# gnss-sdr/gnss-sdr

Hardware: NVIDIA B200
Metric: Msamples/s through N-channel E/P/L correlator (higher is better)
Workload: dtype f32

## Files before the change

### gnss_sdr_b200/csrc/trk_shared_kernel.cu

```cuda
#include "trk_device.cuh"

namespace b200
{
constexpr int kShK = 8;
constexpr int kShTile = 512;
#ifndef SH_STAGES
#define SH_STAGES 4
#endif
#ifndef SH_MINB
#define SH_MINB 3
#endif
constexpr int kShStages = SH_STAGES;
#ifndef SH_STRESS
#define SH_STRESS 0
#endif
#if SH_STRESS
__device__ __forceinline__ void stress_delay(unsigned int salt)
{
    unsigned int h = salt * 2654435761u;
    h ^= h >> 15;
    h *= 2246822519u;
    h ^= h >> 13;
    if ((h & 3u) == 0u) __nanosleep(100u + ((h >> 4) & 1023u));
}
#endif
constexpr int kShTblCap = 1152;
constexpr int kShWin = 256;
constexpr int kShThreads = (kShK + 1) * 32;
constexpr int kShReseed = 64;

namespace
{
struct __align__(128) ShSmem
{
    float2 tiles[kShStages][kShTile];
    float tbl[kShK][kShTblCap];
    unsigned long long full[kShStages];
    unsigned long long empty[kShStages];
    unsigned long long item_start[kShK];
    int item_n[kShK];
    int item_band[kShK];
    unsigned long long hull_start;
    int n_tiles;
    int share;
};

__device__ __forceinline__ unsigned int smem_u32(const void* p) { return static_cast<unsigned int>(__cvta_generic_to_shared(p)); }

__device__ __forceinline__ void mbar_init(unsigned long long* bar, unsigned int count)
{
    asm volatile("mbarrier.init.shared::cta.b64 [%0], %1;" ::"r"(smem_u32(bar)), "r"(count) : "memory");
}
__device__ __forceinline__ void mbar_arrive(unsigned long long* bar)
{
    asm volatile("mbarrier.arrive.shared::cta.b64 _, [%0];" ::"r"(smem_u32(bar)) : "memory");
}
__device__ __forceinline__ void mbar_arrive_expect_tx(unsigned long long* bar, unsigned int bytes)
{
    asm volatile("mbarrier.arrive.expect_tx.shared::cta.b64 _, [%0], %1;" ::"r"(smem_u32(bar)), "r"(bytes) : "memory");
}
__device__ __forceinline__ void mbar_wait(unsigned long long* bar, unsigned int parity)
{
    asm volatile(
        "{\n\t"
        ".reg .pred P1;\n\t"
        "LAB_WAIT:\n\t"
        "mbarrier.try_wait.parity.shared::cta.b64 P1, [%0], %1, %2;\n\t"
        "@P1 bra DONE;\n\t"
        "bra LAB_WAIT;\n\t"
        "DONE:\n\t"
        "}" ::"r"(smem_u32(bar)),
        "r"(parity), "r"(0x989680u)
        : "memory");
}
__device__ __forceinline__ void bulk_g2s(void* smem_dst, const void* gmem_src, unsigned int bytes, unsigned long long* bar)
{
    asm volatile("cp.async.bulk.shared::cluster.global.mbarrier::complete_tx::bytes [%0], [%1], %2, [%3];" ::"r"(smem_u32(smem_dst)),
                 "l"(gmem_src), "r"(bytes), "r"(smem_u32(bar))
                 : "memory");
}

template <int TAPS>
__device__ void warp_correlate_general(const b200_trk_item& it, const ChanDesc& ch, const BandDesc& bd, float2 (&acc)[TAPS])
{
    const int lane = threadIdx.x & 31;
    const unsigned long long s0 = it.sample_index - bd.first_index;
    const unsigned long long T0 = turns_from_rad(-static_cast<double>(it.rem_carrier_phase_rad));
    const unsigned long long DT = turns_from_rad(-static_cast<double>(it.phase_step_rad));
    const int body = (it.n / 8) * 8;
    for (int n = lane; n < it.n; n += 32)
        {
            const float2 x = ldg_stream8(bd.base + ((s0 + static_cast<unsigned long long>(n)) & bd.mask));
            const float2 z = phasor_from_turns(T0 + DT * static_cast<unsigned long long>(n));
            const float wr = fmaf(x.x, z.x, -x.y * z.y);
            const float wi = fmaf(x.x, z.y, x.y * z.x);
            const float nf = static_cast<float>(n);
#pragma unroll
            for (int t = 0; t < TAPS; t++)
                {
                    const int idx = (n < body) ? chip_index_avx(it.code_phase_step_chips, nf, __fsub_rn(ch.shifts[t], it.rem_code_phase_chips))
                                               : chip_index_generic(it.code_phase_step_chips, nf, ch.shifts[t], it.rem_code_phase_chips);
                    const float c = ch.code[mod_pos(idx, ch.code_len)];
                    acc[t].x = fmaf(wr, c, acc[t].x);
                    acc[t].y = fmaf(wi, c, acc[t].y);
                }
        }
}

struct SmemTileLoader
{
    const float4* p;
    __device__ __forceinline__ float4 operator()(int k) const { return p[32 * k]; }
};
struct GlobalTileLoader
{
    const float2* base;
    unsigned long long mask, off, limit;
    __device__ __forceinline__ float4 operator()(int k) const
    {
        const unsigned long long o = off + 64ULL * static_cast<unsigned long long>(k);
        if (mask == ~0ULL && o + 2ULL > limit) return make_float4(0.f, 0.f, 0.f, 0.f);
        return ldg_stream16(base + (o & mask));
    }
};

template <int TAPS, bool MASKED, class Loader>
__device__ __forceinline__ void warp_tile(const Loader& load, float vlo, float vhi, float step, const float2 (&aux2)[TAPS],
    unsigned int tbl_off, float2 Dr2, float2 Di2, float& fa, float& fb, float2& zr, float2& zi, float2 (&are)[TAPS], float2 (&aim)[TAPS])
{
    const float2 magic2 = make_float2(12582912.0f, 12582912.0f);
#pragma unroll
    for (int k = 0; k < kShTile / 64; k++)
        {
            const float4 v = load(k);
            float ua = fa, ub = fb;
            float2 xa = make_float2(v.x, v.y), xb = make_float2(v.z, v.w);
            if (MASKED)
                {
                    if (fa < vlo || fa > vhi) xa = make_float2(0.f, 0.f);
                    if (fb < vlo || fb > vhi) xb = make_float2(0.f, 0.f);
                    ua = fminf(fmaxf(fa, vlo), vhi);
                    ub = fminf(fmaxf(fb, vlo), vhi);
                }
            float2 wr2, wi2;
            wr2.x = fmaf(xa.x, zr.x, -xa.y * zi.x);
            wi2.x = fmaf(xa.x, zi.x, xa.y * zr.x);
            wr2.y = fmaf(xb.x, zr.y, -xb.y * zi.y);
            wi2.y = fmaf(xb.x, zi.y, xb.y * zr.y);
            const float2 m2 = make_float2(__fmul_rn(step, ua), __fmul_rn(step, ub));
#pragma unroll
            for (int t = 0; t < TAPS; t++)
                {
                    const float2 tt = __fadd2_rd(__fadd2_rn(m2, aux2[t]), magic2);
                    const float ca = lds_f32((__float_as_uint(tt.x) << 2) + tbl_off);
                    const float cb = lds_f32((__float_as_uint(tt.y) << 2) + tbl_off);
                    const float2 c2 = make_float2(ca, cb);
                    are[t] = __ffma2_rn(wr2, c2, are[t]);
                    aim[t] = __ffma2_rn(wi2, c2, aim[t]);
                }
            const float2 t1 = __fmul2_rn(zi, Di2);
            const float2 nzr = __ffma2_rn(zr, Dr2, make_float2(-t1.x, -t1.y));
            zi = __ffma2_rn(zr, Di2, __fmul2_rn(zi, Dr2));
            zr = nzr;
            fa += 64.0f;
            fb += 64.0f;
        }
}

template <int TAPS>
__global__ void __launch_bounds__(kShThreads, SH_MINB) trk_shared_kernel(const b200_trk_item* __restrict__ items, int n_items,
    const ChanDesc* __restrict__ chans, const BandDesc* __restrict__ bands, float2* __restrict__ out, int out_stride)
{
    extern __shared__ __align__(128) unsigned char sh_raw[];
    ShSmem& sm = *reinterpret_cast<ShSmem*>(sh_raw);
    const int warp = threadIdx.x >> 5, lane = threadIdx.x & 31;
    const int group = blockIdx.x;
    const int item_id = group * kShK + warp;
    const bool consumer = warp < kShK;
    const bool have_item = consumer && item_id < n_items;

    b200_trk_item it;
    ChanDesc const* ch = nullptr;
    BandDesc bd;
    if (have_item)
        {
            it = items[item_id];
            ch = &chans[it.channel];
            bd = bands[ch->band];
        }
    if (threadIdx.x == 0)
        {
            for (int s = 0; s < kShStages; s++)
                {
                    mbar_init(&sm.full[s], 1);
                    mbar_init(&sm.empty[s], kShK);
                }
            asm volatile("fence.mbarrier_init.release.cluster;" ::: "memory");
        }
    if (consumer && lane == 0)
        {
            sm.item_n[warp] = have_item ? it.n : 0;
            sm.item_band[warp] = have_item ? ch->band : -1;
            sm.item_start[warp] = have_item ? (it.sample_index - bd.first_index) : 0ULL;
        }
    __syncthreads();
    if (threadIdx.x == 0)
        {
            unsigned long long lo = ~0ULL, hi = 0ULL;
            int band = -1, share = 1, nmax = 0;
            for (int w = 0; w < kShK; w++)
                {
                    if (sm.item_n[w] <= 0) continue;
                    if (band < 0) band = sm.item_band[w];
                    if (sm.item_band[w] != band) share = 0;
                    lo = min(lo, sm.item_start[w]);
                    hi = max(hi, sm.item_start[w] + static_cast<unsigned long long>(sm.item_n[w]));
                    nmax = max(nmax, sm.item_n[w]);
                }
            if (band < 0) share = 0;
            lo &= ~1ULL;
            if (share && (hi - lo) > 3ULL * static_cast<unsigned long long>(nmax) + 2ULL * kShTile) share = 0;
            sm.hull_start = lo;
            sm.n_tiles = share ? static_cast<int>((hi - lo + kShTile - 1) / kShTile) : 0;
            sm.share = share;
        }
    __syncthreads();
    const int n_tiles = sm.n_tiles;
    const unsigned long long hull_start = sm.hull_start;

    if (!consumer)
        {
            if (lane == 0 && n_tiles > 0)
                {
                    BandDesc pb;
                    {
                        int w0 = 0;
                        while (sm.item_n[w0] <= 0) w0++;
                        pb = bands[sm.item_band[w0]];
                    }
                    const bool ring = (pb.mask != ~0ULL);
                    const unsigned long long cap = ring ? pb.mask + 1ULL : pb.limit;
                    for (int t = 0; t < n_tiles; t++)
                        {
                            const int s = t % kShStages;
                            const unsigned int par = static_cast<unsigned int>((t / kShStages) & 1);
                            mbar_wait(&sm.empty[s], par ^ 1u);
#if SH_STRESS
                            stress_delay(static_cast<unsigned int>(t) * 31u + blockIdx.x * 7u + 3u);
#endif
                            unsigned long long src = hull_start + static_cast<unsigned long long>(t) * kShTile;
                            unsigned int n1 = kShTile, n2 = 0;
                            if (ring)
                                {
                                    src &= pb.mask;
                                    if (src + kShTile > cap)
                                        {
                                            n1 = static_cast<unsigned int>(cap - src);
                                            n2 = kShTile - n1;
                                        }
                                }
                            else
                                {
                                    if (src >= cap)
                                        n1 = 0;
                                    else if (src + kShTile > cap)
                                        n1 = static_cast<unsigned int>(cap - src) & ~1u;
                                }
                            mbar_arrive_expect_tx(&sm.full[s], (n1 + n2) * 8u);
                            if (n1) bulk_g2s(&sm.tiles[s][0], pb.base + src, n1 * 8u, &sm.full[s]);
                            if (n2) bulk_g2s(&sm.tiles[s][n1], pb.base, n2 * 8u, &sm.full[s]);
                        }
                }
            return;
        }

    float2 acc[TAPS];
#pragma unroll
    for (int t = 0; t < TAPS; t++) acc[t] = make_float2(0.f, 0.f);

    bool table_path = false, whole_table = false;
    unsigned long long my_hull = 0;
    int body = 0, a_i = 0, t_first = 0, t_last = 0;
    float step = 0.f;
    unsigned int tbl_off = 0;
    float2 aux2[TAPS];
    float2 Dr2, Di2, Gr2, Gi2, zr2, zi2, zr, zi;
    unsigned long long T0 = 0, DT = 0;
    if (have_item && it.n > 0)
        {
            body = (it.n / 8) * 8;
            step = it.code_phase_step_chips;
            const float rem = it.rem_code_phase_chips;
            T0 = turns_from_rad(-static_cast<double>(it.rem_carrier_phase_rad));
            DT = turns_from_rad(-static_cast<double>(it.phase_step_rad));
            float smin = ch->shifts[0], smax = ch->shifts[0];
#pragma unroll
            for (int t = 0; t < TAPS; t++)
                {
                    const float sh = ch->shifts[t];
                    const float a2 = __fsub_rn(sh, rem);
                    aux2[t] = make_float2(a2, a2);
                    smin = fminf(smin, sh);
                    smax = fmaxf(smax, sh);
                }
            const float span_bound = ceilf(fabsf(step) * static_cast<float>(kShTile)) + ceilf(smax - smin) + 6.0f;
            table_path = !ch->high_dyn && span_bound <= static_cast<float>(kShWin) && fabsf(step) * static_cast<float>(it.n) < 3.0e6f &&
                         fabsf(smax) < 1.0e5f && fabsf(smin) < 1.0e5f && fabsf(rem) < 1.0e6f;
            if (table_path)
                {
                    {
                        int elo = 0x7fffffff, ehi = -0x7fffffff - 1;
                        const float nl = static_cast<float>(max(body - 1, 0));
#pragma unroll
                        for (int q = 0; q < TAPS; q++)
                            {
                                const int i0 = chip_index_avx(step, 0.f, aux2[q].x);
                                const int i1 = chip_index_avx(step, nl, aux2[q].x);
                                elo = min(elo, min(i0, i1));
                                ehi = max(ehi, max(i0, i1));
                            }
                        whole_table = (static_cast<long long>(ehi) - elo + 3) <= kShTblCap;
                        if (whole_table)
                            {
                                const int wb = elo - 1;
                                const int wspan = ehi - elo + 3;
                                const int L = ch->code_len;
                                int r = mod_pos(wb + lane, L);
                                const int stride = 32 % L;
                                for (int j = lane; j < wspan; j += 32)
                                    {
                                        sm.tbl[warp][j] = __ldg(ch->code + r);
                                        r += stride;
                                        if (r >= L) r -= L;
                                    }
                                asm("sub.u32 %0, %1, %2;" : "=r"(tbl_off) : "r"(smem_u32(&sm.tbl[warp][0])), "r"(4u * (static_cast<unsigned int>(wb) + 0x4B400000u)));
                                __syncwarp();
                            }
                    }
                    my_hull = sm.share ? hull_start : (sm.item_start[warp] & ~1ULL);
                    a_i = static_cast<int>(sm.item_start[warp] - my_hull);
                    t_first = a_i / kShTile;
                    t_last = (a_i + body + kShTile - 1) / kShTile;
                    const float2 D = phasor_from_turns(DT * 64ULL);
                    const float2 G = phasor_from_turns(DT * static_cast<unsigned long long>(64 * kShReseed));
                    Dr2 = make_float2(D.x, D.x);
                    Di2 = make_float2(D.y, D.y);
                    Gr2 = make_float2(G.x, G.x);
                    Gi2 = make_float2(G.y, G.y);
                    const long long n0 = static_cast<long long>(t_first) * kShTile + 2 * lane - a_i;
                    const float2 za = phasor_from_turns(T0 + DT * static_cast<unsigned long long>(n0));
                    const float2 zb = phasor_from_turns(T0 + DT * static_cast<unsigned long long>(n0 + 1));
                    zr2 = make_float2(za.x, zb.x);
                    zi2 = make_float2(za.y, zb.y);
                    zr = zr2;
                    zi = zi2;
                }
        }

    float2 are[TAPS], aim[TAPS];
#pragma unroll
    for (int t = 0; t < TAPS; t++) are[t] = aim[t] = make_float2(0.f, 0.f);
    int tiles_in_group = 0;
    int next_wb = 0;
    float fa = static_cast<float>(t_first * kShTile + 2 * lane - a_i), fb = fa + 1.0f;
    auto process_tile = [&](int t, const auto& load) {
        const int n_tile0 = t * kShTile - a_i;
        const bool interior = (n_tile0 >= 0) && (n_tile0 + kShTile <= body);
        const int n_lo = max(n_tile0, 0), n_hi = min(n_tile0 + kShTile, body) - 1;
        const float vlo = static_cast<float>(n_lo), vhi = static_cast<float>(n_hi);
        if (!whole_table)
            {
                auto stage_window = [&](int tt) {
                    const int m0 = tt * kShTile - a_i;
                    const float lo_f = static_cast<float>(max(m0, 0)), hi_f = static_cast<float>(min(m0 + kShTile, body) - 1);
                    int wlo = 0x7fffffff, whi = -0x7fffffff - 1;
#pragma unroll
                    for (int q = 0; q < TAPS; q++)
                        {
                            const int i0 = chip_index_avx(step, lo_f, aux2[q].x);
                            const int i1 = chip_index_avx(step, hi_f, aux2[q].x);
                            wlo = min(wlo, min(i0, i1));
                            whi = max(whi, max(i0, i1));
                        }
                    const int wb = wlo - 1;
                    const int wspan = min(whi - wlo + 3, kShWin);
                    const int L = ch->code_len;
                    int r = mod_pos(wb + lane, L);
                    const int stride = 32 % L;
                    float* dst = &sm.tbl[warp][(tt & 1) * kShWin];
                    for (int j = lane; j < wspan; j += 32)
                        {
                            asm volatile("cp.async.ca.shared.global [%0], [%1], 4;" ::"r"(smem_u32(dst + j)), "l"(ch->code + r) : "memory");
                            r += stride;
                            if (r >= L) r -= L;
                        }
                    return wb;
                };
                if (t == t_first) next_wb = stage_window(t);
                const int wb = next_wb;
                asm volatile("cp.async.wait_all;" ::: "memory");
                __syncwarp();
                if (t + 1 < t_last) next_wb = stage_window(t + 1);
                asm("sub.u32 %0, %1, %2;" : "=r"(tbl_off) : "r"(smem_u32(&sm.tbl[warp][(t & 1) * kShWin])), "r"(4u * (static_cast<unsigned int>(wb) + 0x4B400000u)));
            }
        if (interior)
            warp_tile<TAPS, false>(load, vlo, vhi, step, aux2, tbl_off, Dr2, Di2, fa, fb, zr, zi, are, aim);
        else
            warp_tile<TAPS, true>(load, vlo, vhi, step, aux2, tbl_off, Dr2, Di2, fa, fb, zr, zi, are, aim);
        if (++tiles_in_group == kShReseed / 8)
            {
                const float2 t2 = __fmul2_rn(zi2, Gi2);
                const float2 ngr = __ffma2_rn(zr2, Gr2, make_float2(-t2.x, -t2.y));
                zi2 = __ffma2_rn(zr2, Gi2, __fmul2_rn(zi2, Gr2));
                zr2 = ngr;
                zr = zr2;
                zi = zi2;
                tiles_in_group = 0;
            }
        __syncwarp();
    };

    for (int t = 0; t < n_tiles; t++)
        {
            const int s = t % kShStages;
            const unsigned int par = static_cast<unsigned int>((t / kShStages) & 1);
            mbar_wait(&sm.full[s], par);
#if SH_STRESS
            stress_delay(static_cast<unsigned int>(t) * 17u + static_cast<unsigned int>(warp) * 101u + blockIdx.x * 13u);
#endif
            if (table_path && t >= t_first && t < t_last)
                {
                    const SmemTileLoader ld{reinterpret_cast<const float4*>(&sm.tiles[s][0]) + lane};
                    process_tile(t, ld);
                }
#if SH_STRESS
            stress_delay(static_cast<unsigned int>(t) * 29u + static_cast<unsigned int>(warp) * 53u + blockIdx.x * 5u + 1u);
            __syncwarp();
#endif
            if (lane == 0) mbar_arrive(&sm.empty[s]);
        }
    if (!sm.share && table_path)
        {
            for (int t = t_first; t < t_last; t++)
                {
                    const GlobalTileLoader ld{bd.base, bd.mask, my_hull + static_cast<unsigned long long>(t) * kShTile + 2ULL * lane, bd.limit};
                    process_tile(t, ld);
                }
        }
    if (have_item && it.n > 0)
        {
            if (table_path)
                {
#pragma unroll
                    for (int t = 0; t < TAPS; t++)
                        {
                            acc[t].x = are[t].x + are[t].y;
                            acc[t].y = aim[t].x + aim[t].y;
                        }
                    const int n = body + lane;
                    if (n < it.n)
                        {
                            const unsigned long long s0 = it.sample_index - bd.first_index;
                            const float2 x = ldg_stream8(bd.base + ((s0 + static_cast<unsigned long long>(n)) & bd.mask));
                            const float2 z = phasor_from_turns(T0 + DT * static_cast<unsigned long long>(n));
                            const float wr = fmaf(x.x, z.x, -x.y * z.y);
                            const float wi = fmaf(x.x, z.y, x.y * z.x);
#pragma unroll
                            for (int t = 0; t < TAPS; t++)
                                {
                                    const int idx = chip_index_generic(step, static_cast<float>(n), ch->shifts[t], it.rem_code_phase_chips);
                                    const float c = __ldg(ch->code + mod_pos(idx, ch->code_len));
                                    acc[t].x = fmaf(wr, c, acc[t].x);
                                    acc[t].y = fmaf(wi, c, acc[t].y);
                                }
                        }
                }
            else
                {
                    warp_correlate_general<TAPS>(it, *ch, bd, acc);
                }
#pragma unroll
            for (int t = 0; t < TAPS; t++)
                {
#pragma unroll
                    for (int o = 16; o > 0; o >>= 1)
                        {
                            acc[t].x += __shfl_xor_sync(0xffffffffu, acc[t].x, o);
                            acc[t].y += __shfl_xor_sync(0xffffffffu, acc[t].y, o);
                        }
                }
            if (lane < TAPS)
                {
                    float2 r = acc[0];
#pragma unroll
                    for (int t = 1; t < TAPS; t++)
                        if (lane == t) r = acc[t];
                    out[static_cast<size_t>(item_id) * out_stride + lane] = r;
                }
        }
    else if (have_item && lane < ch->taps)
        {
            out[static_cast<size_t>(item_id) * out_stride + lane] = make_float2(0.f, 0.f);
        }
}
}

int launch_trk_shared(const b200_trk_item* items, int n_items, const ChanDesc* chans, const BandDesc* bands, float2* out,
    int out_stride, int taps_uniform, cudaStream_t stream)
{
    if (n_items <= 0) return B200_OK;
    const int groups = (n_items + kShK - 1) / kShK;
    static DeviceOnce once;
    const int once_dev = once.begin();
    if (once_dev >= 0)
        {
            B200_CUDA_TRY(cudaFuncSetAttribute(trk_shared_kernel<1>, cudaFuncAttributeMaxDynamicSharedMemorySize, static_cast<int>(sizeof(ShSmem))));
            B200_CUDA_TRY(cudaFuncSetAttribute(trk_shared_kernel<3>, cudaFuncAttributeMaxDynamicSharedMemorySize, static_cast<int>(sizeof(ShSmem))));
            B200_CUDA_TRY(cudaFuncSetAttribute(trk_shared_kernel<5>, cudaFuncAttributeMaxDynamicSharedMemorySize, static_cast<int>(sizeof(ShSmem))));
            once.done(once_dev);
        }
    const size_t smem = sizeof(ShSmem);
    switch (taps_uniform)
        {
        case 1: trk_shared_kernel<1><<<groups, kShThreads, smem, stream>>>(items, n_items, chans, bands, out, out_stride); break;
        case 3: trk_shared_kernel<3><<<groups, kShThreads, smem, stream>>>(items, n_items, chans, bands, out, out_stride); break;
        case 5: trk_shared_kernel<5><<<groups, kShThreads, smem, stream>>>(items, n_items, chans, bands, out, out_stride); break;
        default: return B200_ERR_ARG;
        }
    B200_CUDA_TRY(cudaGetLastError());
    return B200_OK;
}

int trk_shared_max_code_len() { return kShTblCap - 64; }

}
```

Measured before the change: 939,800.

## Add chip-run prefix-sum correlation path with padded cp.async tile staging

Adds a run path in which each lane handles 16 contiguous samples. Within such a run the code phase crosses at most one chip boundary, so each tap is computed as two table lookups plus a prefix-sum lookup, instead of a per-sample lookup and FMA. The carrier rotation is applied once per run, using per-lane rotation factors and a prefix buffer kept in shared memory. To support this, the producer warp's bulk TMA copies are replaced with per-lane 16-byte cp.async into a padded row layout that avoids bank conflicts. The change also cuts per-tap work but adds shared memory and register pressure, with minimum blocks per SM lowered from 3 to 2, and adds rounding-sensitive boundary logic.

```diff
diff --git a/gnss_sdr_b200/csrc/trk_shared_kernel.cu b/gnss_sdr_b200/csrc/trk_shared_kernel.cu
--- a/gnss_sdr_b200/csrc/trk_shared_kernel.cu
+++ b/gnss_sdr_b200/csrc/trk_shared_kernel.cu
@@ -7,8 +7,15 @@
 #ifndef SH_STAGES
 #define SH_STAGES 4
 #endif
+#ifndef SH_CHIPRUN
+#define SH_CHIPRUN 1
+#endif
 #ifndef SH_MINB
+#if SH_CHIPRUN
+#define SH_MINB 2
+#else
 #define SH_MINB 3
+#endif
 #endif
 constexpr int kShStages = SH_STAGES;
 #ifndef SH_STRESS
@@ -28,13 +35,22 @@
 constexpr int kShWin = 256;
 constexpr int kShThreads = (kShK + 1) * 32;
 constexpr int kShReseed = 64;
+constexpr int kShRun = 16;
+constexpr int kShRow = kShRun + 2;
+constexpr float kRunStepMin = 1.0f / 128.0f;
+constexpr float kRunSpanMax = 0.9f;
+constexpr float kRunChipMax = 4096.0f;
 
 namespace
 {
 struct __align__(128) ShSmem
 {
-    float2 tiles[kShStages][kShTile];
+    float2 tiles[kShStages][(kShTile / kShRun) * kShRow];
     float tbl[kShK][kShTblCap];
+#if SH_CHIPRUN
+    float2 pref[kShK][kShRun][32];
+    float4 rot[kShK][kShRun];
+#endif
     unsigned long long full[kShStages];
     unsigned long long empty[kShStages];
     unsigned long long item_start[kShK];
@@ -54,10 +70,6 @@
 __device__ __forceinline__ void mbar_arrive(unsigned long long* bar)
 {
     asm volatile("mbarrier.arrive.shared::cta.b64 _, [%0];" ::"r"(smem_u32(bar)) : "memory");
-}
-__device__ __forceinline__ void mbar_arrive_expect_tx(unsigned long long* bar, unsigned int bytes)
-{
-    asm volatile("mbarrier.arrive.expect_tx.shared::cta.b64 _, [%0], %1;" ::"r"(smem_u32(bar)), "r"(bytes) : "memory");
 }
 __device__ __forceinline__ void mbar_wait(unsigned long long* bar, unsigned int parity)
 {
@@ -73,12 +85,6 @@
         "r"(parity), "r"(0x989680u)
         : "memory");
 }
-__device__ __forceinline__ void bulk_g2s(void* smem_dst, const void* gmem_src, unsigned int bytes, unsigned long long* bar)
-{
-    asm volatile("cp.async.bulk.shared::cluster.global.mbarrier::complete_tx::bytes [%0], [%1], %2, [%3];" ::"r"(smem_u32(smem_dst)),
-                 "l"(gmem_src), "r"(bytes), "r"(smem_u32(bar))
-                 : "memory");
-}
 
 template <int TAPS>
 __device__ void warp_correlate_general(const b200_trk_item& it, const ChanDesc& ch, const BandDesc& bd, float2 (&acc)[TAPS])
@@ -109,8 +115,8 @@
 
 struct SmemTileLoader
 {
-    const float4* p;
-    __device__ __forceinline__ float4 operator()(int k) const { return p[32 * k]; }
+    const float2* p;
+    __device__ __forceinline__ float4 operator()(int k) const { return *reinterpret_cast<const float4*>(p + 4 * kShRow * k); }
 };
 struct GlobalTileLoader
 {
@@ -125,8 +131,8 @@
 };
 
 template <int TAPS, bool MASKED, class Loader>
-__device__ __forceinline__ void warp_tile(const Loader& load, float vlo, float vhi, float step, const float2 (&aux2)[TAPS],
-    unsigned int tbl_off, float2 Dr2, float2 Di2, float& fa, float& fb, float2& zr, float2& zi, float2 (&are)[TAPS], float2 (&aim)[TAPS])
+__device__ __forceinline__ void warp_tile(const Loader& load, float vlo, float vhi, float step, const float (&aux)[TAPS],
+    unsigned int tbl_off, float Dr, float Di, float& fa, float& fb, float2& zr, float2& zi, float2 (&are)[TAPS], float2 (&aim)[TAPS])
 {
     const float2 magic2 = make_float2(12582912.0f, 12582912.0f);
 #pragma unroll
@@ -151,21 +157,88 @@
 #pragma unroll
             for (int t = 0; t < TAPS; t++)
                 {
-                    const float2 tt = __fadd2_rd(__fadd2_rn(m2, aux2[t]), magic2);
+                    const float2 tt = __fadd2_rd(__fadd2_rn(m2, make_float2(aux[t], aux[t])), magic2);
                     const float ca = lds_f32((__float_as_uint(tt.x) << 2) + tbl_off);
                     const float cb = lds_f32((__float_as_uint(tt.y) << 2) + tbl_off);
                     const float2 c2 = make_float2(ca, cb);
                     are[t] = __ffma2_rn(wr2, c2, are[t]);
                     aim[t] = __ffma2_rn(wi2, c2, aim[t]);
                 }
-            const float2 t1 = __fmul2_rn(zi, Di2);
-            const float2 nzr = __ffma2_rn(zr, Dr2, make_float2(-t1.x, -t1.y));
-            zi = __ffma2_rn(zr, Di2, __fmul2_rn(zi, Dr2));
+            const float2 t1 = __fmul2_rn(zi, make_float2(Di, Di));
+            const float2 nzr = __ffma2_rn(zr, make_float2(Dr, Dr), make_float2(-t1.x, -t1.y));
+            zi = __ffma2_rn(zr, make_float2(Di, Di), __fmul2_rn(zi, make_float2(Dr, Dr)));
             zr = nzr;
             fa += 64.0f;
             fb += 64.0f;
         }
 }
+
+struct RunSmemLoader
+{
+    const float2* p;
+    __device__ __forceinline__ float4 operator()(int j) const { return *reinterpret_cast<const float4*>(p + 2 * j); }
+};
+struct RunGlobalLoader
+{
+    const float2* base;
+    unsigned long long mask, off, limit;
+    __device__ __forceinline__ float4 operator()(int j) const
+    {
+        const unsigned long long o = off + 2ULL * static_cast<unsigned long long>(j);
+        if (mask == ~0ULL && o + 2ULL > limit) return make_float4(0.f, 0.f, 0.f, 0.f);
+        return __ldg(reinterpret_cast<const float4*>(base + (o & mask)));
+    }
+};
+
+#if SH_CHIPRUN
+template <int TAPS, bool MASKED, class Loader>
+__device__ __forceinline__ void warp_run(const Loader& load, float vlo, float vhi, float step, float inv_step, const float (&aux)[TAPS],
+    unsigned int tbl_off, const float4* rot, float2 z, float fa, float2* pref, float2 (&acc)[TAPS])
+{
+    const float magic = 12582912.0f;
+    float2 P = make_float2(0.f, 0.f);
+#pragma unroll
+    for (int j = 0; j < kShRun / 2; j++)
+        {
+            const float4 v = load(j);
+            const float4 ea = rot[2 * j], eb = rot[2 * j + 1];
+            float2 xa = make_float2(v.x, v.y), xb = make_float2(v.z, v.w);
+            if (MASKED)
+                {
+                    const float fk = fa + static_cast<float>(2 * j);
+                    if (fk < vlo || fk > vhi) xa = make_float2(0.f, 0.f);
+                    if (fk + 1.0f < vlo || fk + 1.0f > vhi) xb = make_float2(0.f, 0.f);
+                }
+            const float2 ua = __ffma2_rn(make_float2(xa.y, xa.y), make_float2(ea.z, ea.w), __fmul2_rn(make_float2(xa.x, xa.x), make_float2(ea.x, ea.y)));
+            const float2 ub = __ffma2_rn(make_float2(xb.y, xb.y), make_float2(eb.z, eb.w), __fmul2_rn(make_float2(xb.x, xb.x), make_float2(eb.x, eb.y)));
+            pref[64 * j] = P;
+            P = __fadd2_rn(P, ua);
+            pref[64 * j + 32] = P;
+            P = __fadd2_rn(P, ub);
+        }
+    const float ua = MASKED ? fminf(fmaxf(fa, vlo), vhi) : fa;
+    const float ub = MASKED ? fminf(fmaxf(fa + static_cast<float>(kShRun - 1), vlo), vhi) : fa + static_cast<float>(kShRun - 1);
+    const float2 m2 = make_float2(__fmul_rn(step, ua), __fmul_rn(step, ub));
+    const float nb = 0.5f - fa;
+    const float2 zs = make_float2(-z.y, z.x);
+#pragma unroll
+    for (int t = 0; t < TAPS; t++)
+        {
+            const float2 tt = __fadd2_rd(__fadd2_rn(m2, make_float2(aux[t], aux[t])), make_float2(magic, magic));
+            const float c0 = lds_f32((__float_as_uint(tt.x) << 2) + tbl_off);
+            const float c1 = lds_f32((__float_as_uint(tt.y) << 2) + tbl_off);
+            const float F1 = __fsub_rn(tt.y, magic);
+            const float bb = __fadd_ru(fmaf(__fsub_rn(F1, aux[t]), inv_step, nb), magic);
+            const float kc = __fsub_rn(bb, magic + 1.0f);
+            const bool before = __fadd_rn(__fmul_rn(step, __fadd_rn(fa, kc)), aux[t]) >= F1;
+            const unsigned int b = (__float_as_uint(bb) - (before ? 1u : 0u)) & (kShRun - 1);
+            const float2 Pb = pref[32 * b];
+            const float dc = __fsub_rn(c0, c1);
+            const float2 q = __ffma2_rn(make_float2(dc, dc), Pb, __fmul2_rn(make_float2(c1, c1), P));
+            acc[t] = __ffma2_rn(make_float2(q.y, q.y), zs, __ffma2_rn(make_float2(q.x, q.x), z, acc[t]));
+        }
+}
+#endif
 
 template <int TAPS>
 __global__ void __launch_bounds__(kShThreads, SH_MINB) trk_shared_kernel(const b200_trk_item* __restrict__ items, int n_items,
@@ -192,7 +265,7 @@
         {
             for (int s = 0; s < kShStages; s++)
                 {
-                    mbar_init(&sm.full[s], 1);
+                    mbar_init(&sm.full[s], 32);
                     mbar_init(&sm.empty[s], kShK);
                 }
             asm volatile("fence.mbarrier_init.release.cluster;" ::: "memory");
@@ -230,7 +303,7 @@
 
     if (!consumer)
         {
-            if (lane == 0 && n_tiles > 0)
+            if (n_tiles > 0)
                 {
                     BandDesc pb;
                     {
@@ -239,36 +312,28 @@
                         pb = bands[sm.item_band[w0]];
                     }
                     const bool ring = (pb.mask != ~0ULL);
-                    const unsigned long long cap = ring ? pb.mask + 1ULL : pb.limit;
                     for (int t = 0; t < n_tiles; t++)
                         {
                             const int s = t % kShStages;
                             const unsigned int par = static_cast<unsigned int>((t / kShStages) & 1);
                             mbar_wait(&sm.empty[s], par ^ 1u);
 #if SH_STRESS
-                            stress_delay(static_cast<unsigned int>(t) * 31u + blockIdx.x * 7u + 3u);
-#endif
-                            unsigned long long src = hull_start + static_cast<unsigned long long>(t) * kShTile;
-                            unsigned int n1 = kShTile, n2 = 0;
-                            if (ring)
+                            if (lane == 0) stress_delay(static_cast<unsigned int>(t) * 31u + blockIdx.x * 7u + 3u);
+                            __syncwarp();
+#endif
+                            const unsigned long long src = hull_start + static_cast<unsigned long long>(t) * kShTile;
+#pragma unroll
+                            for (int k = 0; k < kShTile / 64; k++)
                                 {
-                                    src &= pb.mask;
-                                    if (src + kShTile > cap)
-                                        {
-                                            n1 = static_cast<unsigned int>(cap - src);
-                                            n2 = kShTile - n1;
-                                        }
+                                    const int c = 32 * k + lane;
+                                    const unsigned long long o = src + 2ULL * static_cast<unsigned long long>(c);
+                                    const unsigned int nbytes = (ring || o + 2ULL <= pb.limit) ? 16u : 0u;
+                                    const float2* g = pb.base + (ring ? (o & pb.mask) : (nbytes ? o : 0ULL));
+                                    asm volatile("cp.async.cg.shared.global [%0], [%1], 16, %2;" ::"r"(smem_u32(&sm.tiles[s][(c >> 3) * kShRow + 2 * (c & 7)])),
+                                                 "l"(g), "r"(nbytes)
+                                                 : "memory");
                                 }
-                            else
-                                {
-                                    if (src >= cap)
-                                        n1 = 0;
-                                    else if (src + kShTile > cap)
-                                        n1 = static_cast<unsigned int>(cap - src) & ~1u;
-                                }
-                            mbar_arrive_expect_tx(&sm.full[s], (n1 + n2) * 8u);
-                            if (n1) bulk_g2s(&sm.tiles[s][0], pb.base + src, n1 * 8u, &sm.full[s]);
-                            if (n2) bulk_g2s(&sm.tiles[s][n1], pb.base, n2 * 8u, &sm.full[s]);
+                            asm volatile("cp.async.mbarrier.arrive.noinc.shared::cta.b64 [%0];" ::"r"(smem_u32(&sm.full[s])) : "memory");
                         }
                 }
             return;
@@ -283,8 +348,14 @@
     int body = 0, a_i = 0, t_first = 0, t_last = 0;
     float step = 0.f;
     unsigned int tbl_off = 0;
-    float2 aux2[TAPS];
-    float2 Dr2, Di2, Gr2, Gi2, zr2, zi2, zr, zi;
+    float aux[TAPS];
+    float Dr, Di, Gr, Gi;
+    float2 zr2, zi2, zr, zi;
+    bool run_path = false;
+#if SH_CHIPRUN
+    float inv_step = 0.f;
+    float2 Gt, zrun;
+#endif
     unsigned long long T0 = 0, DT = 0;
     if (have_item && it.n > 0)
         {
@@ -299,7 +370,7 @@
                 {
                     const float sh = ch->shifts[t];
                     const float a2 = __fsub_rn(sh, rem);
-                    aux2[t] = make_float2(a2, a2);
+                    aux[t] = a2;
                     smin = fminf(smin, sh);
                     smax = fmaxf(smax, sh);
                 }
@@ -314,8 +385,8 @@
 #pragma unroll
                         for (int q = 0; q < TAPS; q++)
                             {
-                                const int i0 = chip_index_avx(step, 0.f, aux2[q].x);
-                                const int i1 = chip_index_avx(step, nl, aux2[q].x);
+                                const int i0 = chip_index_avx(step, 0.f, aux[q]);
+                                const int i1 = chip_index_avx(step, nl, aux[q]);
                                 elo = min(elo, min(i0, i1));
                                 ehi = max(ehi, max(i0, i1));
                             }
@@ -343,10 +414,10 @@
                     t_last = (a_i + body + kShTile - 1) / kShTile;
                     const float2 D = phasor_from_turns(DT * 64ULL);
                     const float2 G = phasor_from_turns(DT * static_cast<unsigned long long>(64 * kShReseed));
-                    Dr2 = make_float2(D.x, D.x);
-                    Di2 = make_float2(D.y, D.y);
-                    Gr2 = make_float2(G.x, G.x);
-                    Gi2 = make_float2(G.y, G.y);
+                    Dr = D.x;
+                    Di = D.y;
+                    Gr = G.x;
+                    Gi = G.y;
                     const long long n0 = static_cast<long long>(t_first) * kShTile + 2 * lane - a_i;
                     const float2 za = phasor_from_turns(T0 + DT * static_cast<unsigned long long>(n0));
                     const float2 zb = phasor_from_turns(T0 + DT * static_cast<unsigned long long>(n0 + 1));
@@ -354,6 +425,24 @@
                     zi2 = make_float2(za.y, zb.y);
                     zr = zr2;
                     zi = zi2;
+#if SH_CHIPRUN
+                    float amax = 0.f;
+#pragma unroll
+                    for (int t = 0; t < TAPS; t++) amax = fmaxf(amax, fabsf(aux[t]));
+                    run_path = sm.share && whole_table && step >= kRunStepMin && step * static_cast<float>(kShRun - 1) <= kRunSpanMax &&
+                               step * static_cast<float>(body + 2 * kShTile) <= kRunChipMax && amax <= kRunChipMax;
+                    if (run_path)
+                        {
+                            inv_step = __frcp_rn(step);
+                            if (lane < kShRun)
+                                {
+                                    const float2 e = phasor_from_turns(DT * static_cast<unsigned long long>(lane));
+                                    sm.rot[warp][lane] = make_float4(e.x, e.y, -e.y, e.x);
+                                }
+                            __syncwarp();
+                            Gt = phasor_from_turns(DT * static_cast<unsigned long long>(kShTile));
+                        }
+#endif
                 }
         }
 
@@ -363,7 +452,7 @@
     int tiles_in_group = 0;
     int next_wb = 0;
     float fa = static_cast<float>(t_first * kShTile + 2 * lane - a_i), fb = fa + 1.0f;
-    auto process_tile = [&](int t, const auto& load) {
+    auto process_tile = [&](int t, const auto& load, const auto& run_load) {
         const int n_tile0 = t * kShTile - a_i;
         const bool interior = (n_tile0 >= 0) && (n_tile0 + kShTile <= body);
         const int n_lo = max(n_tile0, 0), n_hi = min(n_tile0 + kShTile, body) - 1;
@@ -377,8 +466,8 @@
 #pragma unroll
                     for (int q = 0; q < TAPS; q++)
                         {
-                            const int i0 = chip_index_avx(step, lo_f, aux2[q].x);
-                            const int i1 = chip_index_avx(step, hi_f, aux2[q].x);
+                            const int i0 = chip_index_avx(step, lo_f, aux[q]);
+                            const int i1 = chip_index_avx(step, hi_f, aux[q]);
                             wlo = min(wlo, min(i0, i1));
                             whi = max(whi, max(i0, i1));
                         }
@@ -403,15 +492,33 @@
                 if (t + 1 < t_last) next_wb = stage_window(t + 1);
                 asm("sub.u32 %0, %1, %2;" : "=r"(tbl_off) : "r"(smem_u32(&sm.tbl[warp][(t & 1) * kShWin])), "r"(4u * (static_cast<unsigned int>(wb) + 0x4B400000u)));
             }
+#if SH_CHIPRUN
+        if (run_path)
+            {
+                const float fr = static_cast<float>(n_tile0 + kShRun * lane);
+                if (tiles_in_group == 0)
+                    zrun = phasor_from_turns(T0 + DT * static_cast<unsigned long long>(static_cast<long long>(n_tile0 + kShRun * lane)));
+                else
+                    zrun = cmulf(zrun, Gt);
+                float2* pref = &sm.pref[warp][0][lane];
+                if (interior)
+                    warp_run<TAPS, false>(run_load, vlo, vhi, step, inv_step, aux, tbl_off, &sm.rot[warp][0], zrun, fr, pref, are);
+                else
+                    warp_run<TAPS, true>(run_load, vlo, vhi, step, inv_step, aux, tbl_off, &sm.rot[warp][0], zrun, fr, pref, are);
+                if (++tiles_in_group == kShReseed / 8) tiles_in_group = 0;
+                __syncwarp();
+                return;
+            }
+#endif
         if (interior)
-            warp_tile<TAPS, false>(load, vlo, vhi, step, aux2, tbl_off, Dr2, Di2, fa, fb, zr, zi, are, aim);
+            warp_tile<TAPS, false>(load, vlo, vhi, step, aux, tbl_off, Dr, Di, fa, fb, zr, zi, are, aim);
         else
-            warp_tile<TAPS, true>(load, vlo, vhi, step, aux2, tbl_off, Dr2, Di2, fa, fb, zr, zi, are, aim);
+            warp_tile<TAPS, true>(load, vlo, vhi, step, aux, tbl_off, Dr, Di, fa, fb, zr, zi, are, aim);
         if (++tiles_in_group == kShReseed / 8)
             {
-                const float2 t2 = __fmul2_rn(zi2, Gi2);
-                const float2 ngr = __ffma2_rn(zr2, Gr2, make_float2(-t2.x, -t2.y));
-                zi2 = __ffma2_rn(zr2, Gi2, __fmul2_rn(zi2, Gr2));
+                const float2 t2 = __fmul2_rn(zi2, make_float2(Gi, Gi));
+                const float2 ngr = __ffma2_rn(zr2, make_float2(Gr, Gr), make_float2(-t2.x, -t2.y));
+                zi2 = __ffma2_rn(zr2, make_float2(Gi, Gi), __fmul2_rn(zi2, make_float2(Gr, Gr)));
                 zr2 = ngr;
                 zr = zr2;
                 zi = zi2;
@@ -430,8 +537,9 @@
 #endif
             if (table_path && t >= t_first && t < t_last)
                 {
-                    const SmemTileLoader ld{reinterpret_cast<const float4*>(&sm.tiles[s][0]) + lane};
-                    process_tile(t, ld);
+                    const SmemTileLoader ld{&sm.tiles[s][(lane >> 3) * kShRow + 2 * (lane & 7)]};
+                    const RunSmemLoader rld{&sm.tiles[s][lane * kShRow]};
+                    process_tile(t, ld, rld);
                 }
 #if SH_STRESS
             stress_delay(static_cast<unsigned int>(t) * 29u + static_cast<unsigned int>(warp) * 53u + blockIdx.x * 5u + 1u);
@@ -443,8 +551,10 @@
         {
             for (int t = t_first; t < t_last; t++)
                 {
-                    const GlobalTileLoader ld{bd.base, bd.mask, my_hull + static_cast<unsigned long long>(t) * kShTile + 2ULL * lane, bd.limit};
-                    process_tile(t, ld);
+                    const unsigned long long off = my_hull + static_cast<unsigned long long>(t) * kShTile;
+                    const GlobalTileLoader ld{bd.base, bd.mask, off + 2ULL * lane, bd.limit};
+                    const RunGlobalLoader rld{bd.base, bd.mask, off + static_cast<unsigned long long>(kShRun * lane), bd.limit};
+                    process_tile(t, ld, rld);
                 }
         }
     if (have_item && it.n > 0)
@@ -454,8 +564,13 @@
 #pragma unroll
                     for (int t = 0; t < TAPS; t++)
                         {
-                            acc[t].x = are[t].x + are[t].y;
-                            acc[t].y = aim[t].x + aim[t].y;
+                            if (run_path)
+                                acc[t] = are[t];
+                            else
+                                {
+                                    acc[t].x = are[t].x + are[t].y;
+                                    acc[t].y = aim[t].x + aim[t].y;
+                                }
                         }
                     const int n = body + lane;
                     if (n < it.n)
```

New measurement: 1.053 million, median of 6. 12.0% higher.
